# chongkuiqi/S2ANet

Measured on AMD Instinct MI355X. Metric: 1024x1024 DOTA chips/sec (R-50-FPN S2ANet inference), higher is better.
Workload: dtype f16; 1 GPU; BASELINE configs[2]: full R-50-FPN S2ANet inference, batch 8 of 1024x1024 synthetic uint8 chips per GPU; 3 independent batches in flight on 3 HIP streams; global_batch=8, num_classes=15, weights=seeded random init of the reference architecture; odm_cls bias calibrated, nms_candidate_cap=160000, nms_candidates_dropped=0, distinct_input_batches=3, fam_cls_branch=True, hip_graph=False, batches_in_flight=3, parallelism=dp1 (one process per GPU)

## Files before the change

s2anet_amd/csrc/conv_ops.hip:

```cpp
#include <hip/hip_fp16.h>
#include <hip/hip_runtime.h>

#include <algorithm>
#include <cstdlib>
#include <type_traits>

#include "common.hpp"
#include "mfma_common.hpp"

namespace s2a {
namespace {

__global__ void k_pack_weight_frag(const _Float16* __restrict__ w, int O, int C, _Float16* __restrict__ wp,
                                   int taps = 9) {
  int64_t e = (int64_t)blockIdx.x * blockDim.x + threadIdx.x;
  int64_t total = (int64_t)O * C * taps;
  if (e >= total) return;
  const int G = O / 64;
  int j = (int)(e & 7);
  int lane = (int)((e >> 3) & 63);
  int kk = (int)((e >> 9) & 3);
  int mt = (int)((e >> 11) & 1);
  int64_t r = e >> 12;
  int g = (int)(r % G);
// ... 503 lines not shown
#pragma unroll
      for (int c4 = 0; c4 < 4; c4++)
#pragma unroll
        for (int kk = 0; kk < 4; kk++)
#pragma unroll
          for (int j = 0; j < 4; j++)
            if (j < nper) {
              const V bf = *reinterpret_cast<const V*>(s_out + (32 * (nt0 + j) + (lane & 31)) * Cfg::kTailRowB +
                                                       (c4 * 64 + kk * 16 + (lane >> 5) * 8) * 2);
              c2[j] = __builtin_amdgcn_mfma_f32_32x32x16_f16(aw[c4 * 4 + kk], bf, c2[j], 0, 0, 0);
            }
      __syncthreads();
      const int rowb = O3 * 2 + 16;
#pragma unroll
      for (int j = 0; j < 4; j++)
        if (j < nper) {
#pragma unroll
          for (int rq = 0; rq < 4; rq++) {
            using h4 = __attribute__((ext_vector_type(4))) _Float16;
            const int och = mt * 32 + 8 * rq + 4 * (lane >> 5);
            const h4 bq = *reinterpret_cast<const h4*>(ex.chain_b + och);
            h2e lo = {(_Float16)(c2[j][rq * 4] + (float)bq[0]), (_Float16)(c2[j][rq * 4 + 1] + (float)bq[1])};
            h2e hi = {(_Float16)(c2[j][rq * 4 + 2] + (float)bq[2]), (_Float16)(c2[j][rq * 4 + 3] + (float)bq[3])};
            lo = __builtin_elementwise_max(lo, h2e{(_Float16)0.f, (_Float16)0.f});
            hi = __builtin_elementwise_max(hi, h2e{(_Float16)0.f, (_Float16)0.f});
            const h4 v4 = {lo[0], lo[1], hi[0], hi[1]};
            *reinterpret_cast<h4*>(s_out + (32 * (nt0 + j) + (lane & 31)) * rowb + och * 2) = v4;
          }
        }
      __syncthreads();
      const int vpr = O3 / 8;
      for (int idx = tid; idx < Cfg::kPos * vpr; idx += kThreads_) {
        const int pos = idx / vpr, col = idx % vpr;
        const int64_t gp = tile_pos(tile, pos, Cfg::kTH, Ho, Wo, HWo, Ntot);
        if (gp >= 0)
          *reinterpret_cast<V*>(ex.chain_out + gp * O3 + col * 8) = *reinterpret_cast<const V*>(s_out + pos * rowb + col * 16);
      }
    }
    return;
  }
  constexpr int VPR = 8 * OG;
  constexpr int NI = (Cfg::kPos * VPR) / kThreads_;
  const bool relu_u = __builtin_amdgcn_readfirstlane(relu) != 0;
  if (residual) {
    const __amdgpu_buffer_rsrc_t rr = __builtin_amdgcn_make_buffer_rsrc(
        const_cast<T*>(residual), 0, (int)((uint64_t)(res_up ? Ntot / 4 : Ntot) * O * 2), 0x00020000);
    unsigned off[NI];
    V r[NI];
    const int Wr = Wo >> 1;
    const int64_t HWr = (int64_t)(Ho >> 1) * Wr;
#pragma unroll
    for (int i = 0; i < NI; i++) {
      int idx = tid + kThreads_ * i, pos = idx / VPR, col = idx % VPR;
      int64_t gp = TAPS == 9 ? tile_pos(tile, pos, Cfg::kTH, Ho, Wo, HWo, Ntot) : (g0 + pos < Ntot ? g0 + pos : -1);
      const bool ok = gp >= 0 && col * 8 < Oloc;
      off[i] = ok ? (unsigned)((gp * O + o0 + col * 8) * 2) : 0x80000000u;
      unsigned roff = off[i];
      if (res_up && ok) {
        const int64_t bb = gp / HWo, rem = gp % HWo;
        const int yy = (int)(rem / Wo), xx = (int)(rem % Wo);
        roff = (unsigned)(((bb * HWr + (int64_t)(yy >> 1) * Wr + (xx >> 1)) * O + o0 + col * 8) * 2);
      }
      r[i] = __builtin_bit_cast(V, __builtin_amdgcn_raw_buffer_load_b128(rr, (int)roff, 0, 0));
    }
#pragma unroll
    for (int i = 0; i < NI; i++) {
      int idx = tid + kThreads_ * i, pos = idx / VPR, col = idx % VPR;
      V v = *reinterpret_cast<const V*>(s_out + pos * Cfg::kOutRowB + col * 16);
#pragma unroll
      for (int e = 0; e < 8; e += 2) {
        h2e p2 = {(_Float16)((float)v[e] + (float)r[i][e]), (_Float16)((float)v[e + 1] + (float)r[i][e + 1])};
        if (relu_u) p2 = __builtin_elementwise_max(p2, h2e{(_Float16)0.f, (_Float16)0.f});
        v[e] = p2[0];
        v[e + 1] = p2[1];
      }
      if (off[i] != 0x80000000u) *reinterpret_cast<V*>(reinterpret_cast<char*>(out) + off[i]) = v;
    }
  } else {
#pragma unroll
    for (int i = 0; i < NI; i++) {
      int idx = tid + kThreads_ * i, pos = idx / VPR, col = idx % VPR;
      int64_t gp = TAPS == 9 ? tile_pos(tile, pos, Cfg::kTH, Ho, Wo, HWo, Ntot) : (g0 + pos < Ntot ? g0 + pos : -1);
      if (gp >= 0 && col * 8 < Oloc && ex.store_main)
        *reinterpret_cast<V*>(out + gp * O + o0 + col * 8) = *reinterpret_cast<const V*>(s_out + pos * Cfg::kOutRowB + col * 16);
    }
  }
  if constexpr (OG == 4) {
    if (ex.head_w) {
      f32x16 hacc;
#pragma unroll
      for (int r = 0; r < 16; r++) hacc[r] = 0.f;
      const int hpos = 32 * wave + (lane & 31);
      const V* hw = reinterpret_cast<const V*>(ex.head_w) + lane;
#pragma unroll
      for (int c4 = 0; c4 < 4; c4++)
#pragma unroll
        for (int kk = 0; kk < 4; kk++) {
          const V a = hw[(c4 * 8 + kk) * 64];
          const V b = *reinterpret_cast<const V*>(s_out + hpos * Cfg::kOutRowB + (c4 * 64 + kk * 16 + (lane >> 5) * 8) * 2);
          hacc = __builtin_amdgcn_mfma_f32_32x32x16_f16(a, b, hacc, 0, 0, 0);
        }
      const int64_t gp = TAPS == 9 ? tile_pos(tile, hpos, Cfg::kTH, Ho, Wo, HWo, Ntot) : (g0 + hpos < Ntot ? g0 + hpos : -1);
      if (gp >= 0) {
        using h4 = __attribute__((ext_vector_type(4))) _Float16;
#pragma unroll
        for (int rq = 0; rq < 4; rq++) {
          const int och = 8 * rq + 4 * (lane >> 5);
          const h4 hb = *reinterpret_cast<const h4*>(ex.head_b + och);
          h4 v4;
#pragma unroll
          for (int e = 0; e < 4; e++) v4[e] = (_Float16)(hacc[rq * 4 + e] + (float)hb[e]);
          *reinterpret_cast<h4*>(ex.head_out + gp * 64 + och) = v4;
        }
      }
    }
  }
  if (pool_out_) {
    constexpr int GP = 8 * OG;
    for (int item = tid; item < Cfg::kPos * (GP / 8); item += kThreads_) {
      const int pos = item / (GP / 8), q = item % (GP / 8);
      const int64_t gp = TAPS == 9 ? tile_pos(tile, pos, Cfg::kTH, Ho, Wo, HWo, Ntot) : (g0 + pos < Ntot ? g0 + pos : -1);
      if (gp < 0 || q * 64 >= Oloc) continue;
      V res;
#pragma unroll
      for (int e = 0; e < 8; e++) {
        const V v = *reinterpret_cast<const V*>(s_out + pos * Cfg::kOutRowB + (q * 8 + e) * 16);
        _Float16 mx = v[0];
#pragma unroll
        for (int k = 1; k < 8; k++) mx = v[k] > mx ? v[k] : mx;
        res[e] = mx;
      }
      *reinterpret_cast<V*>(pool_out_ + gp * (O / 8) + o0 / 8 + q * 8) = res;
    }
  }
}

template <int CC, int O3>
__global__ __launch_bounds__(256, 2) void k_conv1x1_chain_f16(const _Float16* __restrict__ x,
                                                              const _Float16* __restrict__ wfrag,
                                                              const _Float16* __restrict__ bias,
                                                              const _Float16* __restrict__ residual,
                                                              _Float16* __restrict__ out,
                                                              const _Float16* __restrict__ chain_w,
                                                              const _Float16* __restrict__ chain_b,
                                                              _Float16* __restrict__ chain_out, int64_t Ntot,
                                                              unsigned x_bytes) {
  using T = _Float16;
  using V = f16x8;
  using h2e = __attribute__((ext_vector_type(2))) _Float16;
  using h4e = __attribute__((ext_vector_type(4))) _Float16;
  constexpr int kPos = 64, kChunkB = kPos * kRowBytes, kStRowB = 528;
  constexpr bool C16 = O3 >= 256;
  constexpr int NG3 = C16 ? O3 / 256 : 1;
  constexpr int G3 = O3 / 64;
  extern __shared__ __attribute__((aligned(16))) char smem[];
  const int tid = threadIdx.x, lane = tid & 63, wave = tid >> 6;
  const int wave_u = __builtin_amdgcn_readfirstlane(wave);
  const int64_t tile = xcd_remap(blockIdx.x, gridDim.x);
  const int64_t g0 = tile * kPos;
  constexpr int K = 64 * CC, O = 4 * K, NG = O / 256, G = O / 64;
  char* s_x = smem;
  char* s_st = smem + CC * kChunkB;
  T* s_bias = reinterpret_cast<T*>(s_st + kPos * kStRowB);

  {
    const __amdgpu_buffer_rsrc_t rx = __builtin_amdgcn_make_buffer_rsrc(const_cast<T*>(x), 0, (int)x_bytes, 0x00020000);
    unsigned pvoff[3];
#pragma unroll
    for (int j = 0; j < 3; j++) {
      const int v = (wave_u + 4 * j) * 64 + lane, p = v / 9, q = v % 9;
      const bool in = q < 8 && p < kPos && g0 + p < Ntot;
      pvoff[j] = in ? (unsigned)((g0 + p) * K * 2 + q * 16) : 0x80000000u;
    }
#pragma unroll
    for (int cc = 0; cc < CC; cc++)
#pragma unroll
      for (int j = 0; j < 3; j++) {
        const int i = wave_u + 4 * j;
        if (i < 9)
          __builtin_amdgcn_raw_ptr_buffer_load_lds(rx, (__attribute__((address_space(3))) void*)(s_x + cc * kChunkB + i * 1024), 16,
                                                   (int)pvoff[j], cc * 128, 0, 0);
      }
  }

  const int kg16 = lane >> 4, i16 = lane & 15;
  const int pix16 = (i16 >= 4 && i16 < 12) ? (((i16 - 4) >> 1) * 4 + (i16 & 1))
                                           : (((i16 & 3) >> 1) * 4 + 2 + (i16 & 1) + (i16 >= 12 ? 8 : 0));
  const int bofs = (kg16 & 1) * 64 + (kg16 >> 1) * 16;
  const int wlane = ((lane >> 4) & 1) * 128 + (lane >> 5) * 32 + (lane & 15);
  auto load_w16 = [&](const T* wf, int s, int Gn, int g, int ks, V (&wv)[4]) {
    const V* p = reinterpret_cast<const V*>(wf) + ((int64_t)s * Gn + g) * 8 * 64 + wlane + ks * 64;
#pragma unroll
    for (int a = 0; a < 4; a++) wv[a] = p[(a >> 1) * 4 * 64 + (a & 1) * 16];
  };
  auto mma16 = [&](const char* brow, int tile_b, int ks, const V (&wv)[4], f32x4 (&acc)[4][4]) {
    V pf[4];
#pragma unroll
    for (int b = 0; b < 4; b++) pf[b] = *reinterpret_cast<const V*>(brow + b * tile_b + ks * 32);
#pragma unroll
    for (int a = 0; a < 4; a++)
#pragma unroll
      for (int b = 0; b < 4; b++) acc[a][b] = __builtin_amdgcn_mfma_f32_16x16x32_f16(wv[a], pf[b], acc[a][b], 0, 0, 0);
  };

  f32x4 cacc[C16 ? NG3 : 1][4][4];
  f32x16 c2[2];
  if constexpr (C16) {
#pragma unroll
    for (int n = 0; n < NG3; n++)
#pragma unroll
      for (int a = 0; a < 4; a++)
#pragma unroll
        for (int b = 0; b < 4; b++)
#pragma unroll
          for (int r = 0; r < 4; r++) cacc[n][a][b][r] = 0.f;
  } else {
#pragma unroll
    for (int j = 0; j < 2; j++)
#pragma unroll
      for (int r = 0; r < 16; r++) c2[j][r] = 0.f;
  }
  const bool has_res = residual != nullptr;
  const __amdgpu_buffer_rsrc_t rr = __builtin_amdgcn_make_buffer_rsrc(const_cast<T*>(has_res ? residual : out), 0,
                                                                      (int)((uint64_t)Ntot * O * 2), 0x00020000);
  const int pos0 = tid >> 5, col0 = tid & 31;
  const int nvalid = (int)(Ntot - g0 < kPos ? Ntot - g0 : kPos);
  const unsigned off0 = (unsigned)(((g0 + pos0) * O + col0 * 8) * 2);
  __syncthreads();

#pragma unroll 1
  for (int gi = 0; gi < NG; gi++) {
    const int o0 = gi * 256;
    s_bias[tid] = bias[o0 + tid];
    f32x4 acc[4][4];
#pragma unroll
    for (int a = 0; a < 4; a++)
#pragma unroll
      for (int b = 0; b < 4; b++)
#pragma unroll
        for (int r = 0; r < 4; r++) acc[a][b][r] = 0.f;
    {
      V w[2][4];
      load_w16(wfrag, 0, G, gi * 4 + wave, 0, w[0]);
#pragma unroll
      for (int st = 0; st < 2 * CC; st++) {
        if (st + 1 < 2 * CC) load_w16(wfrag, (st + 1) >> 1, G, gi * 4 + wave, (st + 1) & 1, w[(st + 1) & 1]);
        mma16(s_x + (st >> 1) * kChunkB + pix16 * kRowBytes + bofs, 16 * kRowBytes, st & 1, w[st & 1], acc);
        __builtin_amdgcn_sched_barrier(0);
      }
    }
    const unsigned offg = off0 + o0 * 2;
    V r8[8];
    if (has_res) {
#pragma unroll
      for (int i = 0; i < 8; i++)
        r8[i] = __builtin_bit_cast(V, __builtin_amdgcn_raw_buffer_load_b128(
                                          rr, (int)(pos0 + 8 * i < nvalid ? offg + i * (8 * O * 2) : 0x80000000u), 0, 0));
    }
    __syncthreads();
#pragma unroll
    for (int a = 0; a < 4; a++) {
      const int och = wave * 64 + 16 * a + 4 * kg16;
      const h4e bq = *reinterpret_cast<const h4e*>(s_bias + och);
#pragma unroll
      for (int b = 0; b < 4; b++) {
        h2e lo = {(_Float16)(acc[a][b][0] + (float)bq[0]), (_Float16)(acc[a][b][1] + (float)bq[1])};
        h2e hi = {(_Float16)(acc[a][b][2] + (float)bq[2]), (_Float16)(acc[a][b][3] + (float)bq[3])};
        if (!has_res) {
          lo = __builtin_elementwise_max(lo, h2e{(_Float16)0.f, (_Float16)0.f});
          hi = __builtin_elementwise_max(hi, h2e{(_Float16)0.f, (_Float16)0.f});
        }
        *reinterpret_cast<h4e*>(s_st + (16 * b + pix16) * kStRowB + och * 2) = h4e{lo[0], lo[1], hi[0], hi[1]};
      }
    }
    __syncthreads();
    V aw[C16 ? 4 : 16];
    if constexpr (C16) {
      load_w16(chain_w, gi * 4, G3, wave, 0, aw);
    } else {
      const V* cwp = reinterpret_cast<const V*>(chain_w) + lane + ((wave >> 1) * 8 + (wave & 1) * 4) * 64;
#pragma unroll
      for (int c4 = 0; c4 < 4; c4++)
#pragma unroll
        for (int kk = 0; kk < 4; kk++) aw[c4 * 4 + kk] = cwp[((int64_t)(gi * 4 + c4) * G3 * 8 + kk) * 64];
    }
#pragma unroll
    for (int i = 0; i < 8; i++) {
      const int pos = pos0 + 8 * i, col = col0;
      V v = *reinterpret_cast<const V*>(s_st + pos * kStRowB + col * 16);
      if (has_res) {
#pragma unroll
        for (int e = 0; e < 8; e += 2) {
          h2e p2 = {(_Float16)((float)v[e] + (float)r8[i][e]), (_Float16)((float)v[e + 1] + (float)r8[i][e + 1])};
          p2 = __builtin_elementwise_max(p2, h2e{(_Float16)0.f, (_Float16)0.f});
          v[e] = p2[0];
          v[e + 1] = p2[1];
        }
        *reinterpret_cast<V*>(s_st + pos * kStRowB + col * 16) = v;
      }
      if (pos < nvalid) *reinterpret_cast<V*>(reinterpret_cast<char*>(out) + (offg + i * (8 * O * 2))) = v;
    }
    __syncthreads();
    if constexpr (C16) {
      V w2[4];
#pragma unroll
      for (int st = 0; st < NG3 * 8; st++) {
        constexpr int kLast = NG3 * 8 - 1;
        const int nx = st + 1;
        if (st < kLast) load_w16(chain_w, gi * 4 + ((nx >> 1) & 3), G3, wave + 4 * (nx >> 3), nx & 1, (st & 1) ? aw : w2);
        mma16(s_st + pix16 * kStRowB + ((st >> 1) & 3) * 128 + bofs, 16 * kStRowB, st & 1, (st & 1) ? w2 : aw, cacc[st >> 3]);
        __builtin_amdgcn_sched_barrier(0);
      }
    } else {
#pragma unroll
      for (int c4 = 0; c4 < 4; c4++)
#pragma unroll
        for (int kk = 0; kk < 4; kk++)
#pragma unroll
          for (int j = 0; j < 2; j++) {
            const V bf = *reinterpret_cast<const V*>(s_st + (32 * j + (lane & 31)) * kStRowB + (c4 * 64 + kk * 16 + (lane >> 5) * 8) * 2);
            c2[j] = __builtin_amdgcn_mfma_f32_32x32x16_f16(aw[c4 * 4 + kk], bf, c2[j], 0, 0, 0);
          }
    }
  }
  __syncthreads();
  constexpr int rowb = O3 * 2 + 16;
  if constexpr (C16) {
#pragma unroll
    for (int n = 0; n < NG3; n++)
#pragma unroll
      for (int a = 0; a < 4; a++) {
        const int och = (wave + 4 * n) * 64 + 16 * a + 4 * kg16;
        const h4e bq = *reinterpret_cast<const h4e*>(chain_b + och);
#pragma unroll
        for (int b = 0; b < 4; b++) {
          h2e lo = {(_Float16)(cacc[n][a][b][0] + (float)bq[0]), (_Float16)(cacc[n][a][b][1] + (float)bq[1])};
          h2e hi = {(_Float16)(cacc[n][a][b][2] + (float)bq[2]), (_Float16)(cacc[n][a][b][3] + (float)bq[3])};
          lo = __builtin_elementwise_max(lo, h2e{(_Float16)0.f, (_Float16)0.f});
          hi = __builtin_elementwise_max(hi, h2e{(_Float16)0.f, (_Float16)0.f});
          *reinterpret_cast<h4e*>(smem + (16 * b + pix16) * rowb + och * 2) = h4e{lo[0], lo[1], hi[0], hi[1]};
        }
      }
  } else {
#pragma unroll
    for (int j = 0; j < 2; j++)
#pragma unroll
      for (int rq = 0; rq < 4; rq++) {
        const int och = wave * 32 + 8 * rq + 4 * (lane >> 5);
        const h4e bq = *reinterpret_cast<const h4e*>(chain_b + och);
        h2e lo = {(_Float16)(c2[j][rq * 4] + (float)bq[0]), (_Float16)(c2[j][rq * 4 + 1] + (float)bq[1])};
        h2e hi = {(_Float16)(c2[j][rq * 4 + 2] + (float)bq[2]), (_Float16)(c2[j][rq * 4 + 3] + (float)bq[3])};
        lo = __builtin_elementwise_max(lo, h2e{(_Float16)0.f, (_Float16)0.f});
        hi = __builtin_elementwise_max(hi, h2e{(_Float16)0.f, (_Float16)0.f});
        *reinterpret_cast<h4e*>(smem + (32 * j + (lane & 31)) * rowb + och * 2) = h4e{lo[0], lo[1], hi[0], hi[1]};
      }
  }
  __syncthreads();
  constexpr int vpr = O3 / 8;
#pragma unroll
  for (int i = 0; i < kPos * vpr / 256; i++) {
    const int idx = tid + 256 * i, pos = idx / vpr, col = idx % vpr;
    if (g0 + pos < Ntot)
      *reinterpret_cast<V*>(chain_out + (g0 + pos) * O3 + col * 8) = *reinterpret_cast<const V*>(smem + pos * rowb + col * 16);
  }
}

constexpr int kNarrowPatch = ConvCfg<9, 1>::kPatchBytes;
constexpr int kNarrowJ = ConvCfg<9, 1>::kJ;
constexpr int kNarrowDma = ConvCfg<9, 1>::kDma;
constexpr int kNarrowOutBytes = 128 * 32;
constexpr int kNarrowFixedLds = 3 * kNarrowPatch + 2 * kNarrowOutBytes + 64;
constexpr int kNarrowMaxC = 256;
inline int narrow_lds_bytes(int C) { return kNarrowFixedLds + (C / 64) * 9 * 2048; }

__global__ __launch_bounds__(256, 1) void k_conv3x3_narrow_f16(const _Float16* __restrict__ x,
                                                               const _Float16* __restrict__ wfrag,
                                                               const _Float16* __restrict__ bias,
                                                               _Float16* __restrict__ out, int C, int O_used, int relu,
                                                               unsigned x_bytes, LevelTab lt, int tiles) {
  using T = _Float16;
  using V = f16x8;
  using h2e = __attribute__((ext_vector_type(2))) _Float16;
  using h4e = __attribute__((ext_vector_type(4))) _Float16;
  extern __shared__ __attribute__((aligned(16))) char smem[];
  const int tid = threadIdx.x, lane = tid & 63, wave = tid >> 6;
  const int wave_u = __builtin_amdgcn_readfirstlane(wave);
  const int CC = C / 64, nstage = 9 * CC;
  char* s_w = smem + 3 * kNarrowPatch;
  char* s_out = s_w + nstage * 2048;
  T* s_bias = reinterpret_cast<T*>(s_out + 2 * kNarrowOutBytes);
  const int t_begin = (int)((int64_t)blockIdx.x * tiles / gridDim.x);
  const int t_end = (int)((int64_t)(blockIdx.x + 1) * tiles / gridDim.x);
  if (t_begin >= t_end) return;
  const unsigned row_bytes = (unsigned)C * 2;
  const __amdgpu_buffer_rsrc_t rx = __builtin_amdgcn_make_buffer_rsrc(const_cast<T*>(x), 0, (int)x_bytes, 0x00020000);

  struct Tile { int H, W, ty0, tx0; int64_t base; };
  auto decode = [&](int tile) {
    int t0 = 0, p0 = 0, H = lt.H[0], W = lt.W[0];
#pragma unroll
    for (int i = 1; i < kMaxLevels; i++)
      if (i < lt.n && tile >= lt.tile0[i]) {
        t0 = lt.tile0[i]; p0 = lt.pix0[i]; H = lt.H[i]; W = lt.W[i];
      }
    const int txn = (W + 15) / 16, tyn = (H + 7) / 8, loc = tile - t0;
    const int bimg = loc / (txn * tyn), trem = loc % (txn * tyn);
    return Tile{H, W, (trem / txn) * 8, (trem % txn) * 16, (int64_t)p0 + (int64_t)bimg * H * W};
  };
  unsigned pvoff[kNarrowJ];
  auto bind = [&](const Tile& tl) {
#pragma unroll
    for (int j = 0; j < kNarrowJ; j++) {
      const int v = (wave_u + 4 * j) * 64 + lane, p = v / 9, q = v % 9;
      const int yy = tl.ty0 - 1 + p / kCPW, xx = tl.tx0 - 1 + p % kCPW;
      const bool in = q < 8 && p < ConvCfg<9, 1>::kPix && yy >= 0 && yy < tl.H && xx >= 0 && xx < tl.W;
      pvoff[j] = in ? (unsigned)((tl.base + (int64_t)yy * tl.W + xx) * row_bytes + q * 16) : 0x80000000u;
    }
  };
  auto piece_issue = [&](int buf, int cc, int j) {
    const int i = wave_u + 4 * j;
    if (i < kNarrowDma)
      __builtin_amdgcn_raw_ptr_buffer_load_lds(rx, (__attribute__((address_space(3))) void*)(smem + buf * kNarrowPatch + i * 1024),
                                               16, (int)pvoff[j], cc * 128, 0, 0);
  };
  auto patch_issue = [&](int buf, int cc) {
#pragma unroll
    for (int j = 0; j < kNarrowJ; j++) piece_issue(buf, cc, j);
  };

  int itile = t_begin, icc = 0;
  bool ivalid = true;
  auto advance = [&]() {
    if (++icc == CC) {
      icc = 0;
      if (++itile < t_end) bind(decode(itile)); else ivalid = false;
    }
  };
  bind(decode(t_begin));
  patch_issue(0, 0);
  advance();
  if (ivalid) {
    patch_issue(1, icc);
    advance();
  }
  for (int idx = tid; idx < nstage * 128; idx += 256) {
    const int s = idx >> 7, ks = (idx >> 6) & 1, l = idx & 63;
    *reinterpret_cast<V*>(s_w + idx * 16) =
        reinterpret_cast<const V*>(wfrag)[(int64_t)s * 512 + ks * 64 + ((l >> 4) & 1) * 128 + (l >> 5) * 32 + (l & 15)];
  }
  if (tid < 16) s_bias[tid] = (bias && tid < O_used) ? bias[tid] : (T)0.f;

  const int kg16 = lane >> 4, i16 = lane & 15;
  const int pix16 = (i16 >= 4 && i16 < 12) ? (((i16 - 4) >> 1) * 4 + (i16 & 1))
                                           : (((i16 & 3) >> 1) * 4 + 2 + (i16 & 1) + (i16 >= 12 ? 8 : 0));
  const int fbase16 = (2 * wave * kCPW + pix16) * kRowBytes + (kg16 & 1) * 64 + (kg16 >> 1) * 16;
  constexpr int kTile16 = kCPW * kRowBytes;
  const bool relu_u = __builtin_amdgcn_readfirstlane(relu) != 0;
  f32x4 acc[2];
#pragma unroll
  for (int b = 0; b < 2; b++)
#pragma unroll
    for (int r = 0; r < 4; r++) acc[b][r] = 0.f;
  __syncthreads();

  auto stage_sync = [&](bool issued) {
    __builtin_amdgcn_sched_barrier(0);
    if (!issued) asm volatile("s_waitcnt vmcnt(0) lgkmcnt(0)\n\ts_barrier" ::: "memory");
    else if (wave_u + 4 * (kNarrowJ - 1) < kNarrowDma) asm volatile("s_waitcnt vmcnt(7) lgkmcnt(0)\n\ts_barrier" ::: "memory");
    else asm volatile("s_waitcnt vmcnt(6) lgkmcnt(0)\n\ts_barrier" ::: "memory");
    __builtin_amdgcn_sched_barrier(0);
  };
  static_assert(kNarrowJ == 7 && kNarrowDma == 26, "stage_sync counts 7 pieces on waves 0-1 and 6 on waves 2-3");
  int rb = 0;
  for (int tile = t_begin; tile < t_end; tile++) {
    const Tile cur = decode(tile);
    bool issued = false;
    for (int cc = 0; cc < CC; cc++) {
      const bool more = ivalid;
      issued = more;
      const int ncc = icc, wb = rb == 0 ? 2 : rb - 1, buf = rb;
      const char* P = smem + buf * kNarrowPatch + fbase16;
      const char* Wc = s_w + cc * (9 * 2048) + lane * 16;
      V fa[3][2], fp[3][2][2];
      auto load_tap = [&](int t, V (&a)[2], V (&p)[2][2]) {
        const int toff = ((t / 3) * kCPW + (t % 3)) * kRowBytes;
#pragma unroll
        for (int ks = 0; ks < 2; ks++) {
          a[ks] = *reinterpret_cast<const V*>(Wc + (t * 2 + ks) * 1024);
          p[ks][0] = *reinterpret_cast<const V*>(P + toff + ks * 32);
          p[ks][1] = *reinterpret_cast<const V*>(P + kTile16 + toff + ks * 32);
        }
      };
      load_tap(0, fa[0], fp[0]);
      load_tap(1, fa[1], fp[1]);
#pragma unroll
      for (int t = 0; t < 9; t++) {
        if (t + 2 < 9) load_tap(t + 2, fa[(t + 2) % 3], fp[(t + 2) % 3]);
        if (t < kNarrowJ && more) piece_issue(wb, ncc, t);
#pragma unroll
        for (int ks = 0; ks < 2; ks++) {
          acc[0] = __builtin_amdgcn_mfma_f32_16x16x32_f16(fa[t % 3][ks], fp[t % 3][ks][0], acc[0], 0, 0, 0);
          acc[1] = __builtin_amdgcn_mfma_f32_16x16x32_f16(fa[t % 3][ks], fp[t % 3][ks][1], acc[1], 0, 0, 0);
// ... 98 lines not shown
    S2A_CONV_FORM(9, 4, 1, 1, 0, 1);
    S2A_CONV_FORM(9, 2, 1, 1, 0, 1);
    S2A_CONV_FORM(9, 4, 1, 1, 0, 0);
    S2A_CONV_FORM(9, 2, 1, 1, 0, 0);
    S2A_CONV_FORM(9, 1, 1, 1, 0, 0);
    S2A_CONV_FORM(1, 4, 1, 2, 0, 0);
    S2A_CONV_FORM(1, 4, 1, 1, 0, 0);
    S2A_CONV_FORM(1, 2, 1, 1, 0, 0);
    S2A_CONV_FORM(1, 1, 1, 1, 0, 0);
    S2A_CONV_FORM(9, 1, 2, 1, 1, 0);
    S2A_CONV_FORM(9, 1, 1, 1, 1, 0);
#undef S2A_CONV_FORM
    s2a::set_error("conv: no kernel of form <%d, %d, %d, %d, %d, %d>", f.taps, f.og, f.ph, f.sd, f.tail, f.ht);
    return S2A_EINVAL;
  }
};

inline int env_ph(const char* name, int ph) {
  const char* f = getenv(name);
  return f ? (atoi(f) == 2 ? 2 : 1) : ph;
}
inline bool env_flag(const char* name, bool on) {
  const char* f = getenv(name);
  return f ? atoi(f) != 0 : on;
}
inline int conv_og(int64_t out_channels) { return out_channels % 256 == 0 ? 4 : (out_channels % 128 == 0 ? 2 : 1); }

ConvForm conv_form_nhwc(int64_t batch, int64_t channels, int64_t height, int64_t width, int64_t out_channels, int ksize,
                        int stride) {
  const int64_t Ho = (height - 1) / stride + 1, Wo = (width - 1) / stride + 1;
  const int og = conv_og(out_channels);
  const int64_t groups = (out_channels + 64 * og - 1) / (64 * og);
  if (ksize == 3 && stride == 2) return {9, og == 4 ? 4 : 2, 1, 2, 0, 0};
  if (ksize == 3 && og < 4 && channels % 64 == 0) {
    const int64_t tiles16 = batch * ((Wo + 15) / 16) * ((Ho + 15) / 16) * groups;
    if (env_ph("S2A_CONV_PH_NARROW", tiles16 >= 256 ? 2 : 1) == 2) return {9, og, 2, 1, 0, 0};
  }
  if (ksize == 3 && og == 4 && channels % 64 == 0) {
    const int64_t tiles16 = batch * ((Wo + 15) / 16) * ((Ho + 15) / 16) * groups;
    if (env_ph("S2A_CONV_PH", tiles16 >= 512 ? 2 : 1) == 2) return {9, 4, 2, 1, 0, 0};
  }
  if (ksize == 3 && og >= 2) {
    const int64_t wgs128 = batch * ((Wo + 15) / 16) * ((Ho + 7) / 8) * groups;
    if (env_flag("S2A_CONV3_HALF", wgs128 < 256)) return {9, og, 1, 1, 0, 1};
  }
  if (ksize == 3) return {9, og, 1, 1, 0, 0};
  if (og == 4) {
    const int64_t wgs128 = (batch * Ho * Wo + 127) / 128 * groups;
    if (env_flag("S2A_CONV1_HALF", wgs128 < 256)) return {1, 4, 1, 2, 0, 0};
  }
  return {1, og, 1, 1, 0, 0};
}

ConvForm conv_form_up2(int64_t out_channels) { return {1, conv_og(out_channels), 1, 1, 0, 0}; }

ConvForm conv_form_pyramid(int64_t channels, int64_t out_channels, bool has_head) {
  int og = conv_og(out_channels);
  const char* og_env = getenv("S2A_CONV_OG");
  if (og_env && !has_head) og = std::min(og, std::max(1, atoi(og_env)));
  if (og == 3) og = 1;
  const int ph = (og == 4 && channels % 64 == 0) ? env_ph("S2A_CONV_PH", 2) : 1;
  return {9, og, ph, 1, 0, 0};
}

ConvForm conv_form_tail(int64_t batch, int64_t height, int64_t width) {
  const int64_t tiles16 = batch * ((width + 15) / 16) * ((height + 15) / 16);
  return {9, 1, env_ph("S2A_CONV_PH_NARROW", tiles16 >= 256 ? 2 : 1), 1, 1, 0};
}

int conv_nhwc_check_sizes(int64_t batch, int64_t channels, int64_t height, int64_t width, int64_t out_channels, int ksize,
                          int stride, bool has_residual) {
  S2A_CHECK_ARG(batch >= 0 && channels > 0 && out_channels > 0 && height > 0 && width > 0, "conv: bad shape");
  S2A_CHECK_ARG(ksize == 3 || ksize == 1, "conv: kernel size must be 1 or 3");
  S2A_CHECK_ARG(stride == 1 || stride == 2, "conv: stride must be 1 or 2");
  S2A_CHECK_ARG(!(ksize == 3 && stride == 2) || out_channels % 128 == 0, "conv: 3x3 stride 2 needs out_channels % 128 == 0");
  S2A_CHECK_ARG((channels % 64 == 0 || channels == 32) && out_channels % 64 == 0,
                "conv: channels must be 32 or a multiple of 64, out_channels a multiple of 64");
  const uint64_t x_bytes = (uint64_t)batch * height * width * channels * 2;
  S2A_CHECK_ARG(x_bytes < (1ull << 31) && (ksize == 1 || (height < 32000 && width < 32000)),
                "conv: input too large for 32-bit offsets");
  S2A_CHECK_ARG(!has_residual || (uint64_t)batch * ((height - 1) / stride + 1) * ((width - 1) / stride + 1) * out_channels * 2 < (1ull << 31),
                "conv: output too large for the fused residual (32-bit offsets)");
  return S2A_OK;
}
}
}

extern "C" int s2a_conv_nhwc_f16_form(int64_t batch, int64_t channels, int64_t height, int64_t width, int64_t out_channels,
                                      int ksize, int stride, int32_t form[6]) {
  if (int rc = conv_nhwc_check_sizes(batch, channels, height, width, out_channels, ksize, stride, false)) return rc;
  S2A_CHECK_ARG(form, "conv_form: NULL form");
  const ConvForm f = conv_form_nhwc(batch, channels, height, width, out_channels, ksize, stride);
  form[0] = f.taps, form[1] = f.og, form[2] = f.ph, form[3] = f.sd, form[4] = f.tail, form[5] = f.ht;
  return S2A_OK;
}

extern "C" int s2a_conv_nhwc_f16(const void* x, const void* weight_frag, const void* bias, const void* residual,
                                 void* out, int64_t batch, int64_t channels, int64_t height, int64_t width,
                                 int64_t out_channels, int ksize, int stride, int relu, s2a_stream_t stream) {
  if (int rc = conv_nhwc_check_sizes(batch, channels, height, width, out_channels, ksize, stride, residual != nullptr)) return rc;
  if (batch == 0) return S2A_OK;
  S2A_CHECK_ARG(x && weight_frag && out, "conv: NULL tensor");
  S2A_CHECK_ARG(((uintptr_t)x % 16) == 0 && ((uintptr_t)out % 16) == 0 && ((uintptr_t)weight_frag % 16) == 0 &&
                ((uintptr_t)bias % 8) == 0 && ((uintptr_t)residual % 16) == 0, "conv: tensors must be 16-byte aligned");
  const int Ho = (int)((height - 1) / stride + 1), Wo = (int)((width - 1) / stride + 1);
  const ConvCall c{(const _Float16*)x, (const _Float16*)weight_frag, (const _Float16*)bias, (const _Float16*)residual,
                   (_Float16*)out, batch, (int)channels, (int)height, (int)width, Ho, Wo, stride, (int)out_channels, relu,
                   as_stream(stream)};
  return c.run(conv_form_nhwc(batch, channels, height, width, out_channels, ksize, stride));
}

extern "C" int s2a_conv3x3_tail1x1_f16(const void* x, const void* weight_frag, const void* bias,
                                       const void* tail_weight_frag, const void* tail_bias, const void* residual,
                                       void* out, const void* chain_weight_frag, const void* chain_bias, void* chain_out,
                                       int64_t chain_channels, int64_t batch, int64_t channels, int64_t mid_channels,
                                       int64_t out_channels, int64_t height, int64_t width, s2a_stream_t stream) {
  S2A_CHECK_ARG(batch >= 0 && height > 0 && width > 0, "conv3x3_tail1x1: bad shape");
  S2A_CHECK_ARG(channels == 64 && mid_channels == 64 && out_channels == 256,
                "conv3x3_tail1x1: built for the 64 -> 64 -> 256 bottleneck tail");
  S2A_CHECK_ARG((uint64_t)batch * height * width * out_channels * 2 < (1ull << 31) && height < 32000 && width < 32000,
                "conv3x3_tail1x1: tensor too large for 32-bit offsets");
  if (batch == 0) return S2A_OK;
  S2A_CHECK_ARG(x && weight_frag && bias && tail_weight_frag && tail_bias && out, "conv3x3_tail1x1: NULL tensor");
  S2A_CHECK_ARG(((uintptr_t)x % 16) == 0 && ((uintptr_t)out % 16) == 0 && ((uintptr_t)weight_frag % 16) == 0 &&
                ((uintptr_t)tail_weight_frag % 16) == 0 && ((uintptr_t)bias % 8) == 0 && ((uintptr_t)tail_bias % 8) == 0 &&
                ((uintptr_t)residual % 16) == 0, "conv3x3_tail1x1: tensors must be 16-byte aligned");
  ConvExtra ex{};
  ex.store_main = 0;
  ex.tail_w = (const _Float16*)tail_weight_frag;
  ex.tail_b = (const _Float16*)tail_bias;
  ex.tail_res = (const _Float16*)residual;
  ex.tail_out = (_Float16*)out;
  if (chain_weight_frag || chain_bias || chain_out) {
    S2A_CHECK_ARG(chain_weight_frag && chain_bias && chain_out, "conv3x3_tail1x1: chain filter, bias and output go together");
    S2A_CHECK_ARG(chain_channels == 64 || chain_channels == 128, "conv3x3_tail1x1: the chained 1x1 has 64 or 128 maps");
    S2A_CHECK_ARG(((uintptr_t)chain_weight_frag % 16) == 0 && ((uintptr_t)chain_bias % 8) == 0 && ((uintptr_t)chain_out % 16) == 0,
                  "conv3x3_tail1x1: chain tensors must be 16-byte aligned");
    ex.chain_w = (const _Float16*)chain_weight_frag;
    ex.chain_b = (const _Float16*)chain_bias;
    ex.chain_out = (_Float16*)chain_out;
    ex.chain_O = (int)chain_channels;
  }
  const ConvCall c{(const _Float16*)x, (const _Float16*)weight_frag, (const _Float16*)bias, nullptr, (_Float16*)out, batch, 64,
                   (int)height, (int)width, (int)height, (int)width, 1, 64, 1, as_stream(stream), nullptr, 0, 0, ex};
  return c.run(conv_form_tail(batch, height, width));
}

namespace s2a {
namespace {
template <int CC, int O3>
int launch_conv1x1_chain(const _Float16* x, const _Float16* wfrag, const _Float16* bias, const _Float16* residual, _Float16* out,
                         const _Float16* cw, const _Float16* cb, _Float16* cout, int64_t P, hipStream_t st) {
  constexpr int K = 64 * CC;
  const int loop = CC * 64 * kRowBytes + 64 * 528 + 512;
  const int tail = 64 * (O3 * 2 + 16);
  const int lds = loop > tail ? loop : tail;
  auto kern = k_conv1x1_chain_f16<CC, O3>;
  S2A_HIP(hipFuncSetAttribute(reinterpret_cast<const void*>(kern), hipFuncAttributeMaxDynamicSharedMemorySize, lds));
  kern<<<dim3((unsigned)((P + 63) / 64)), 256, lds, st>>>(x, wfrag, bias, residual, out, cw, cb, cout, P,
                                                          (unsigned)((uint64_t)P * K * 2));
  S2A_LAUNCH_CHECK();
  return S2A_OK;
}
}
}

extern "C" int s2a_conv1x1_chain_f16(const void* x, const void* weight_frag, const void* bias, const void* residual,
                                     void* out, const void* chain_weight_frag, const void* chain_bias, void* chain_out,
                                     int64_t chain_channels, int64_t batch, int64_t channels, int64_t out_channels,
                                     int64_t height, int64_t width, s2a_stream_t stream) {
  S2A_CHECK_ARG(batch >= 0 && height > 0 && width > 0, "conv1x1_chain: bad shape");
  S2A_CHECK_ARG((channels == 128 && out_channels == 512 && (chain_channels == 128 || chain_channels == 256)) ||
                (channels == 256 && out_channels == 1024 && chain_channels == 256),
                "conv1x1_chain: built for (K, O, O3) = (128, 512, 128), (128, 512, 256), (256, 1024, 256)");
  S2A_CHECK_ARG((uint64_t)batch * height * width * out_channels * 2 < (1ull << 31),
                "conv1x1_chain: tensor too large for 32-bit offsets");
  S2A_CHECK_ARG((chain_weight_frag && chain_bias && chain_out) || (!chain_weight_frag && !chain_bias && !chain_out),
                "conv1x1_chain: chain filter, bias and output go together");
  if (batch == 0) return S2A_OK;
  S2A_CHECK_ARG(x && weight_frag && bias && out && chain_weight_frag, "conv1x1_chain: NULL tensor");
  S2A_CHECK_ARG(((uintptr_t)x % 16) == 0 && ((uintptr_t)out % 16) == 0 && ((uintptr_t)weight_frag % 16) == 0 &&
                ((uintptr_t)bias % 8) == 0 && ((uintptr_t)residual % 16) == 0 && ((uintptr_t)chain_weight_frag % 16) == 0 &&
                ((uintptr_t)chain_bias % 8) == 0 && ((uintptr_t)chain_out % 16) == 0,
                "conv1x1_chain: tensors must be 16-byte aligned");
  const int64_t P = batch * height * width;
  const _Float16 *X = (const _Float16*)x, *Wf = (const _Float16*)weight_frag, *Bi = (const _Float16*)bias,
                 *R = (const _Float16*)residual, *Cw = (const _Float16*)chain_weight_frag, *Cb = (const _Float16*)chain_bias;
  hipStream_t st = as_stream(stream);
  if (channels == 256) return launch_conv1x1_chain<4, 256>(X, Wf, Bi, R, (_Float16*)out, Cw, Cb, (_Float16*)chain_out, P, st);
  if (chain_channels == 128) return launch_conv1x1_chain<2, 128>(X, Wf, Bi, R, (_Float16*)out, Cw, Cb, (_Float16*)chain_out, P, st);
  return launch_conv1x1_chain<2, 256>(X, Wf, Bi, R, (_Float16*)out, Cw, Cb, (_Float16*)chain_out, P, st);
}

extern "C" int s2a_conv1x1_add_up2_f16(const void* x, const void* weight_frag, const void* bias, const void* coarse,
                                       void* out, int64_t batch, int64_t channels, int64_t height, int64_t width,
                                       int64_t out_channels, s2a_stream_t stream) {
  S2A_CHECK_ARG(batch >= 0 && channels > 0 && out_channels > 0 && height > 0 && width > 0, "conv_add_up2: bad shape");
  S2A_CHECK_ARG(height % 2 == 0 && width % 2 == 0, "conv_add_up2: the map must be exactly twice the coarse map");
  S2A_CHECK_ARG(channels % 64 == 0 && out_channels % 64 == 0, "conv_add_up2: channel counts must be multiples of 64");
  const uint64_t x_bytes = (uint64_t)batch * height * width * channels * 2;
  S2A_CHECK_ARG(x_bytes < (1ull << 31) && (uint64_t)batch * height * width * out_channels * 2 < (1ull << 31),
                "conv_add_up2: tensor too large for 32-bit offsets");
  if (batch == 0) return S2A_OK;
  S2A_CHECK_ARG(x && weight_frag && coarse && out, "conv_add_up2: NULL tensor");
  S2A_CHECK_ARG(((uintptr_t)x % 16) == 0 && ((uintptr_t)out % 16) == 0 && ((uintptr_t)weight_frag % 16) == 0 &&
                ((uintptr_t)bias % 2) == 0 && ((uintptr_t)coarse % 16) == 0, "conv_add_up2: tensors must be 16-byte aligned");
  const ConvCall c{(const _Float16*)x, (const _Float16*)weight_frag, (const _Float16*)bias, (const _Float16*)coarse,
                   (_Float16*)out, batch, (int)channels, (int)height, (int)width, (int)height, (int)width, 1, (int)out_channels, 0,
                   as_stream(stream), nullptr, 0, 1};
  return c.run(conv_form_up2(out_channels));
}

extern "C" int s2a_conv_pack_weight_f16(const void* weight, int64_t out_channels, int64_t channels, int ksize,
                                        void* packed, s2a_stream_t stream) {
  S2A_CHECK_ARG(ksize == 3 || ksize == 1, "conv_pack_weight: kernel size must be 1 or 3");
  S2A_CHECK_ARG(out_channels % 64 == 0 && channels % 64 == 0, "conv_pack_weight: channel counts must be multiples of 64");
  S2A_CHECK_ARG(weight && packed, "conv_pack_weight: NULL tensor");
  const int taps = ksize * ksize;
  const int64_t wtot = out_channels * channels * taps;
  k_pack_weight_frag<<<(unsigned)((wtot + 255) / 256), 256, 0, as_stream(stream)>>>(
      (const _Float16*)weight, (int)out_channels, (int)channels, (_Float16*)packed, taps);
  S2A_LAUNCH_CHECK();
  return S2A_OK;
}

extern "C" int64_t s2a_pyramid_pixels(const s2a_pyramid* pyr, int64_t batch) {
  LevelTab lt; int64_t pix = 0;
  return build_levels(pyr, batch, &lt, &pix) < 0 ? -1 : pix;
}

static int conv3x3_pyramid_impl(const void* x, const void* weight_frag, const void* bias, const void* residual,
                                void* out, ConvExtra ex, int64_t batch, int64_t channels, int64_t out_channels,
                                int relu, const s2a_pyramid* pyr, s2a_stream_t stream);

extern "C" int s2a_conv3x3_pyramid_f16(const void* x, const void* weight_frag, const void* bias, const void* residual,
                                       void* out, int64_t batch, int64_t channels, int64_t out_channels,
                                       int relu, const s2a_pyramid* pyr, s2a_stream_t stream) {
  return conv3x3_pyramid_impl(x, weight_frag, bias, residual, out, ConvExtra{nullptr, nullptr, nullptr, nullptr, 1}, batch,
                              channels, out_channels, relu, pyr, stream);
}

extern "C" int s2a_conv3x3_head_pyramid_f16(const void* x, const void* weight_frag, const void* bias, void* out,
                                            const void* head_weight_frag, const void* head_bias, void* head_out,
                                            int64_t batch, int64_t channels, int64_t out_channels, int relu,
                                            const s2a_pyramid* pyr, s2a_stream_t stream) {
  S2A_CHECK_ARG(out_channels == 256, "conv3x3_head_pyramid: the fused 1x1 head needs a 256-channel tower");
  S2A_CHECK_ARG(head_weight_frag && head_bias && head_out, "conv3x3_head_pyramid: NULL head tensor");
  S2A_CHECK_ARG(((uintptr_t)head_weight_frag % 16) == 0 && ((uintptr_t)head_bias % 8) == 0 && ((uintptr_t)head_out % 16) == 0,
                "conv3x3_head_pyramid: misaligned head tensor");
  ConvExtra ex{nullptr, (const _Float16*)head_weight_frag, (const _Float16*)head_bias, (_Float16*)head_out, out != nullptr};
  return conv3x3_pyramid_impl(x, weight_frag, bias, nullptr, out ? out : head_out, ex, batch, channels, out_channels, relu,
                              pyr, stream);
}

extern "C" int s2a_orconv_pool_pyramid_f16(const void* x, const void* weight_frag, const void* bias, void* out,
                                           void* pooled, int64_t batch, int64_t channels, int64_t out_channels,
                                           const s2a_pyramid* pyr, s2a_stream_t stream) {
  S2A_CHECK_ARG(pooled != nullptr && ((uintptr_t)pooled % 16) == 0 && out_channels % 64 == 0,
                "orconv_pool_pyramid: pooled must be a 16-byte aligned buffer, out_channels a multiple of 64");
  return conv3x3_pyramid_impl(x, weight_frag, bias, nullptr, out, ConvExtra{(_Float16*)pooled, nullptr, nullptr, nullptr, 1},
                              batch, channels, out_channels, 0, pyr, stream);
}

static int conv3x3_pyramid_impl(const void* x, const void* weight_frag, const void* bias, const void* residual,
                                void* out, ConvExtra ex, int64_t batch, int64_t channels, int64_t out_channels,
                                int relu, const s2a_pyramid* pyr, s2a_stream_t stream) {
  S2A_CHECK_ARG(batch >= 0 && channels > 0 && out_channels > 0, "conv_pyramid: bad shape");
  S2A_CHECK_ARG((channels % 64 == 0 || channels == 32) && out_channels % 64 == 0,
                "conv_pyramid: channels must be 32 or a multiple of 64, out_channels a multiple of 64");
  LevelTab lt; int64_t pix = 0;
  const ConvForm form = conv_form_pyramid(channels, out_channels, ex.head_w != nullptr);
  const int64_t tiles = build_levels(pyr, batch, &lt, &pix, 8 * form.ph);
  S2A_CHECK_ARG(tiles >= 0, "conv_pyramid: bad level table (1..8 levels, positive sizes)");
  S2A_CHECK_ARG((uint64_t)pix * channels * 2 < (1ull << 31), "conv_pyramid: input too large for 32-bit offsets");
  if (batch == 0) return S2A_OK;
  S2A_CHECK_ARG(x && weight_frag && out, "conv_pyramid: NULL tensor");
  S2A_CHECK_ARG(((uintptr_t)x % 16) == 0 && ((uintptr_t)out % 16) == 0 && ((uintptr_t)weight_frag % 16) == 0 &&
                ((uintptr_t)bias % 8) == 0 && ((uintptr_t)residual % 16) == 0, "conv_pyramid: tensors must be 16-byte aligned");
  if (lt.n == 1) lt.n = 2, lt.tile0[1] = 0x7fffffff;
  const ConvCall c{(const _Float16*)x, (const _Float16*)weight_frag, (const _Float16*)bias, (const _Float16*)residual,
                   (_Float16*)out, batch, (int)channels, lt.H[0], lt.W[0], lt.H[0], lt.W[0], 1, (int)out_channels, relu,
                   as_stream(stream), &lt, tiles, 0, ex};
  return c.run(form);
}

extern "C" int s2a_conv3x3_narrow_pyramid_f16(const void* x, const void* weight_frag, const void* bias, void* out,
                                              int64_t batch, int64_t channels, int64_t out_channels_used, int relu,
                                              const s2a_pyramid* pyr, s2a_stream_t stream) {
  S2A_CHECK_ARG(batch >= 0 && channels > 0, "conv_narrow_pyramid: bad shape");
  S2A_CHECK_ARG(channels % 64 == 0, "conv_narrow_pyramid: channels must be a multiple of 64");
  S2A_CHECK_ARG(out_channels_used >= 1 && out_channels_used <= 16, "conv_narrow_pyramid: 1..16 maps (out_channels_used)");
  bool narrow = channels <= kNarrowMaxC;
  if (const char* f = getenv("S2A_CONV_NARROW")) narrow = narrow && atoi(f) != 0;
  if (!narrow)
    return conv3x3_pyramid_impl(x, weight_frag, bias, nullptr, out, ConvExtra{nullptr, nullptr, nullptr, nullptr, 1}, batch,
                                channels, 64, relu, pyr, stream);
  LevelTab lt; int64_t pix = 0;
  const int64_t tiles = build_levels(pyr, batch, &lt, &pix, 8);
  S2A_CHECK_ARG(tiles >= 0, "conv_narrow_pyramid: bad level table (1..8 levels, positive sizes)");
  S2A_CHECK_ARG((uint64_t)pix * channels * 2 < (1ull << 31), "conv_narrow_pyramid: input too large for 32-bit offsets");
  if (batch == 0) return S2A_OK;
  S2A_CHECK_ARG(x && weight_frag && out, "conv_narrow_pyramid: NULL tensor");
  S2A_CHECK_ARG(((uintptr_t)x % 16) == 0 && ((uintptr_t)out % 16) == 0 && ((uintptr_t)weight_frag % 16) == 0 &&
                ((uintptr_t)bias % 8) == 0, "conv_narrow_pyramid: tensors must be 16-byte aligned");
  int64_t grid = std::min<int64_t>(tiles, 256);
  if (const char* f = getenv("S2A_CONV_NARROW_WGS")) grid = std::min<int64_t>(grid, std::max(1, atoi(f)));
  const int lds = narrow_lds_bytes((int)channels);
// ... 10 lines not shown
```

Measured before the change: 1976 chips/s.

## Deepen weight prefetch pipeline and preload biases in fused 1x1 conv chain

Reworks the fused 1x1 bottleneck chain kernel so weight fragments are fetched through buffer loads with a three-deep ring for the main GEMM and a four-deep ring for the chained GEMM. The next output group's first weights are prefetched during the epilogue. All main and chain biases are staged into LDS once up front instead of per group, and residual loads and output stores use precomputed buffer offsets so out-of-range rows are masked by the buffer hardware. The aim is to hide global weight-load latency behind MFMA work, at the cost of more registers and a larger LDS allocation, which may lower occupancy.

New measurement: 1990 chips/s (median of 6 runs). Within noise of the previous version (+0.7%).

```diff
diff --git a/s2anet_amd/csrc/conv_ops.hip b/s2anet_amd/csrc/conv_ops.hip
--- a/s2anet_amd/csrc/conv_ops.hip
+++ b/s2anet_amd/csrc/conv_ops.hip
@@ -679,6 +679,7 @@
   constexpr int kPos = 64, kChunkB = kPos * kRowBytes, kStRowB = 528;
   constexpr bool C16 = O3 >= 256;
   constexpr int NG3 = C16 ? O3 / 256 : 1;
+  constexpr int MR = 3, CR = 4;
   constexpr int G3 = O3 / 64;
   extern __shared__ __attribute__((aligned(16))) char smem[];
   const int tid = threadIdx.x, lane = tid & 63, wave = tid >> 6;
@@ -715,11 +716,23 @@
                                            : (((i16 & 3) >> 1) * 4 + 2 + (i16 & 1) + (i16 >= 12 ? 8 : 0));
   const int bofs = (kg16 & 1) * 64 + (kg16 >> 1) * 16;
   const int wlane = ((lane >> 4) & 1) * 128 + (lane >> 5) * 32 + (lane & 15);
-  auto load_w16 = [&](const T* wf, int s, int Gn, int g, int ks, V (&wv)[4]) {
-    const V* p = reinterpret_cast<const V*>(wf) + ((int64_t)s * Gn + g) * 8 * 64 + wlane + ks * 64;
-#pragma unroll
-    for (int a = 0; a < 4; a++) wv[a] = p[(a >> 1) * 4 * 64 + (a & 1) * 16];
+  const __amdgpu_buffer_rsrc_t rw = __builtin_amdgcn_make_buffer_rsrc(const_cast<T*>(wfrag), 0, O * K * 2, 0x00020000);
+  const __amdgpu_buffer_rsrc_t rc = __builtin_amdgcn_make_buffer_rsrc(const_cast<T*>(chain_w), 0, O3 * O * 2, 0x00020000);
+  const int wl16 = wlane * 16;
+  auto load_w16 = [&](__amdgpu_buffer_rsrc_t r, int s, int Gn, int g, int ks, V (&wv)[4]) {
+    const int so = ((s * Gn + g) * 8 * 64 + ks * 64) * 16;
+#pragma unroll
+    for (int a = 0; a < 4; a++)
+      wv[a] = __builtin_bit_cast(V, __builtin_amdgcn_raw_buffer_load_b128(r, wl16 + (a & 1) * 256, so + (a >> 1) * 4096, 0));
   };
+  auto load_main = [&](__amdgpu_buffer_rsrc_t r, int gi, int st, V (&wv)[4]) {
+    load_w16(r, st >> 1, G, gi * 4 + wave_u, st & 1, wv);
+  };
+  V w[MR][4];
+#pragma unroll
+  for (int st = 0; st < MR - 1; st++) load_main(rw, 0, st, w[st]);
+  if (tid < O / 4) reinterpret_cast<h4e*>(s_bias)[tid] = reinterpret_cast<const h4e*>(bias)[tid];
+  if (tid < O3 / 4) reinterpret_cast<h4e*>(s_bias + O)[tid] = reinterpret_cast<const h4e*>(chain_b)[tid];
   auto mma16 = [&](const char* brow, int tile_b, int ks, const V (&wv)[4], f32x4 (&acc)[4][4]) {
     V pf[4];
 #pragma unroll
@@ -749,16 +762,19 @@
   }
   const bool has_res = residual != nullptr;
   const __amdgpu_buffer_rsrc_t rr = __builtin_amdgcn_make_buffer_rsrc(const_cast<T*>(has_res ? residual : out), 0,
-                                                                      (int)((uint64_t)Ntot * O * 2), 0x00020000);
+                                                                      has_res ? (int)((uint64_t)Ntot * O * 2) : 0, 0x00020000);
+  const __amdgpu_buffer_rsrc_t ro = __builtin_amdgcn_make_buffer_rsrc(out, 0, (int)((uint64_t)Ntot * O * 2), 0x00020000);
   const int pos0 = tid >> 5, col0 = tid & 31;
   const int nvalid = (int)(Ntot - g0 < kPos ? Ntot - g0 : kPos);
-  const unsigned off0 = (unsigned)(((g0 + pos0) * O + col0 * 8) * 2);
+  unsigned voff[8];
+#pragma unroll
+  for (int i = 0; i < 8; i++)
+    voff[i] = pos0 + 8 * i < nvalid ? (unsigned)(((g0 + pos0 + 8 * i) * O + col0 * 8) * 2) : 0x80000000u;
   __syncthreads();
 
 #pragma unroll 1
   for (int gi = 0; gi < NG; gi++) {
     const int o0 = gi * 256;
-    s_bias[tid] = bias[o0 + tid];
     f32x4 acc[4][4];
 #pragma unroll
     for (int a = 0; a < 4; a++)
@@ -766,29 +782,21 @@
       for (int b = 0; b < 4; b++)
 #pragma unroll
         for (int r = 0; r < 4; r++) acc[a][b][r] = 0.f;
-    {
-      V w[2][4];
-      load_w16(wfrag, 0, G, gi * 4 + wave, 0, w[0]);
-#pragma unroll
-      for (int st = 0; st < 2 * CC; st++) {
-        if (st + 1 < 2 * CC) load_w16(wfrag, (st + 1) >> 1, G, gi * 4 + wave, (st + 1) & 1, w[(st + 1) & 1]);
-        mma16(s_x + (st >> 1) * kChunkB + pix16 * kRowBytes + bofs, 16 * kRowBytes, st & 1, w[st & 1], acc);
-        __builtin_amdgcn_sched_barrier(0);
-      }
-    }
-    const unsigned offg = off0 + o0 * 2;
+#pragma unroll
+    for (int st = 0; st < 2 * CC; st++) {
+      if (st + MR - 1 < 2 * CC) load_main(rw, gi, st + MR - 1, w[(st + MR - 1) % MR]);
+      __builtin_amdgcn_sched_barrier(0);
+      mma16(s_x + (st >> 1) * kChunkB + pix16 * kRowBytes + bofs, 16 * kRowBytes, st & 1, w[st % MR], acc);
+      __builtin_amdgcn_sched_barrier(0);
+    }
     V r8[8];
-    if (has_res) {
-#pragma unroll
-      for (int i = 0; i < 8; i++)
-        r8[i] = __builtin_bit_cast(V, __builtin_amdgcn_raw_buffer_load_b128(
-                                          rr, (int)(pos0 + 8 * i < nvalid ? offg + i * (8 * O * 2) : 0x80000000u), 0, 0));
-    }
+#pragma unroll
+    for (int i = 0; i < 8; i++) r8[i] = __builtin_bit_cast(V, __builtin_amdgcn_raw_buffer_load_b128(rr, (int)voff[i], o0 * 2, 0));
     __syncthreads();
 #pragma unroll
     for (int a = 0; a < 4; a++) {
       const int och = wave * 64 + 16 * a + 4 * kg16;
-      const h4e bq = *reinterpret_cast<const h4e*>(s_bias + och);
+      const h4e bq = *reinterpret_cast<const h4e*>(s_bias + o0 + och);
 #pragma unroll
       for (int b = 0; b < 4; b++) {
         h2e lo = {(_Float16)(acc[a][b][0] + (float)bq[0]), (_Float16)(acc[a][b][1] + (float)bq[1])};
@@ -801,15 +809,27 @@
       }
     }
     __syncthreads();
-    V aw[C16 ? 4 : 16];
+    {
+      const __amdgpu_buffer_rsrc_t rn =
+          __builtin_amdgcn_make_buffer_rsrc(const_cast<T*>(wfrag), 0, gi + 1 < NG ? O * K * 2 : 0, 0x00020000);
+#pragma unroll
+      for (int st = 0; st < MR - 1; st++) load_main(rn, gi + 1, st, w[st]);
+    }
+    V cw[C16 ? CR : 1][4], aw[C16 ? 1 : 16];
+    auto load_c16 = [&](int st, V (&wv)[4]) {
+      load_w16(rc, gi * 4 + ((st >> 1) & 3), G3, wave_u + 4 * (st >> 3), st & 1, wv);
+    };
     if constexpr (C16) {
-      load_w16(chain_w, gi * 4, G3, wave, 0, aw);
+#pragma unroll
+      for (int st = 0; st < CR; st++) load_c16(st, cw[st]);
     } else {
-      const V* cwp = reinterpret_cast<const V*>(chain_w) + lane + ((wave >> 1) * 8 + (wave & 1) * 4) * 64;
+      const int so = ((wave_u >> 1) * 8 + (wave_u & 1) * 4) * 1024;
 #pragma unroll
       for (int c4 = 0; c4 < 4; c4++)
 #pragma unroll
-        for (int kk = 0; kk < 4; kk++) aw[c4 * 4 + kk] = cwp[((int64_t)(gi * 4 + c4) * G3 * 8 + kk) * 64];
+        for (int kk = 0; kk < 4; kk++)
+          aw[c4 * 4 + kk] = __builtin_bit_cast(V, __builtin_amdgcn_raw_buffer_load_b128(
+                                                      rc, lane * 16, so + ((gi * 4 + c4) * G3 * 8 + kk) * 1024, 0));
     }
 #pragma unroll
     for (int i = 0; i < 8; i++) {
@@ -825,17 +845,14 @@
         }
         *reinterpret_cast<V*>(s_st + pos * kStRowB + col * 16) = v;
       }
-      if (pos < nvalid) *reinterpret_cast<V*>(reinterpret_cast<char*>(out) + (offg + i * (8 * O * 2))) = v;
+      __builtin_amdgcn_raw_buffer_store_b128(__builtin_bit_cast(u32x4, v), ro, (int)voff[i], o0 * 2, 0);
     }
     __syncthreads();
     if constexpr (C16) {
-      V w2[4];
 #pragma unroll
       for (int st = 0; st < NG3 * 8; st++) {
-        constexpr int kLast = NG3 * 8 - 1;
-        const int nx = st + 1;
-        if (st < kLast) load_w16(chain_w, gi * 4 + ((nx >> 1) & 3), G3, wave + 4 * (nx >> 3), nx & 1, (st & 1) ? aw : w2);
-        mma16(s_st + pix16 * kStRowB + ((st >> 1) & 3) * 128 + bofs, 16 * kStRowB, st & 1, (st & 1) ? w2 : aw, cacc[st >> 3]);
+        mma16(s_st + pix16 * kStRowB + ((st >> 1) & 3) * 128 + bofs, 16 * kStRowB, st & 1, cw[st % CR], cacc[st >> 3]);
+        if (st + CR < NG3 * 8) load_c16(st + CR, cw[st % CR]);
         __builtin_amdgcn_sched_barrier(0);
       }
     } else {
@@ -858,7 +875,7 @@
 #pragma unroll
       for (int a = 0; a < 4; a++) {
         const int och = (wave + 4 * n) * 64 + 16 * a + 4 * kg16;
-        const h4e bq = *reinterpret_cast<const h4e*>(chain_b + och);
+        const h4e bq = *reinterpret_cast<const h4e*>(s_bias + O + och);
 #pragma unroll
         for (int b = 0; b < 4; b++) {
           h2e lo = {(_Float16)(cacc[n][a][b][0] + (float)bq[0]), (_Float16)(cacc[n][a][b][1] + (float)bq[1])};
@@ -874,7 +891,7 @@
 #pragma unroll
       for (int rq = 0; rq < 4; rq++) {
         const int och = wave * 32 + 8 * rq + 4 * (lane >> 5);
-        const h4e bq = *reinterpret_cast<const h4e*>(chain_b + och);
+        const h4e bq = *reinterpret_cast<const h4e*>(s_bias + O + och);
         h2e lo = {(_Float16)(c2[j][rq * 4] + (float)bq[0]), (_Float16)(c2[j][rq * 4 + 1] + (float)bq[1])};
         h2e hi = {(_Float16)(c2[j][rq * 4 + 2] + (float)bq[2]), (_Float16)(c2[j][rq * 4 + 3] + (float)bq[3])};
         lo = __builtin_elementwise_max(lo, h2e{(_Float16)0.f, (_Float16)0.f});
@@ -1279,7 +1296,7 @@
 int launch_conv1x1_chain(const _Float16* x, const _Float16* wfrag, const _Float16* bias, const _Float16* residual, _Float16* out,
                          const _Float16* cw, const _Float16* cb, _Float16* cout, int64_t P, hipStream_t st) {
   constexpr int K = 64 * CC;
-  const int loop = CC * 64 * kRowBytes + 64 * 528 + 512;
+  const int loop = CC * 64 * kRowBytes + 64 * 528 + (4 * K + O3) * 2;
   const int tail = 64 * (O3 * 2 + 16);
   const int lds = loop > tail ? loop : tail;
   auto kern = k_conv1x1_chain_f16<CC, O3>;
```
